# Superjie13/StereoTracking

Measured on AMD Instinct MI355X. Metric: stereo frame-pairs/sec @1280x720 D=192, higher is better.
Workload: dtype f32; 1 GPU; configs[1]: batch=8 synthetic 1280x720 stereo pairs per GPU, D=192, full YOLOX-s two-branch backbone+PAFPN+head, cost volume at 1/4 res (48 levels) + 2 3x3 aggregation convs + soft-argmin, decode+NMS, per-box depth; global_batch=8, inflight_contexts=4, distinct_input_batches=4, gpu_max_hw_queues=4, hip_force_dev_kernarg=1, parallelism=single process, no process group (no collective in the step), collectives_issued=0, tuning_plan=configs/tuning/mi355x.json, max_det=1000, detections_overflow=False

## Files before the change

include/stereotrack.h:

```cpp
#ifndef STEREOTRACK_H_
#define STEREOTRACK_H_

#include <stddef.h>
#include <stdint.h>

#ifdef __cplusplus
extern "C" {
#endif

#define ST_VERSION 430

enum {
  ST_OK = 0,
  ST_ERR_INVALID = -1,
  ST_ERR_HIP = -2,
  ST_ERR_STATE = -3,
  ST_ERR_WORKSPACE = -4,
  ST_ERR_NOTFOUND = -5
};

typedef void* st_stream_t;

int st_version(void);
const char* st_last_error(void);

typedef struct StConvDesc {
  const float* in_dev;
  int N, Hi, Wi, Cin, in_ld, in_off;
  const float* wgt_dev;
  const float* bias_dev;
  int Cout, KH, KW, stride, pad;
  float* out1_dev;
  int out1_ld, out1_off, split;
  float* out2_dev;
  int out2_ld, out2_off;
  float* up_dev;
  int up_ld, up_off;
  const float* res_dev;
  int res_ld, res_off;
  float post_scale;
  int act;
  const float* wgt_wino_dev;
} StConvDesc;

int st_conv2d_nhwc(const StConvDesc* d, st_stream_t stream);
int st_conv2d_nhwc_variant(const StConvDesc* d, st_stream_t stream, int variant);
size_t st_wino_packed_floats(int Cout, int Cin);
int st_wino_pack_weights(const float* packed_wgt_host, int Cout, int Cin, float* out_host);
int st_conv3x3_wino_group(const StConvDesc* descs, int n, st_stream_t stream);

int st_conv1x1_chain(const StConvDesc* a, const StConvDesc* b, st_stream_t stream);
size_t st_front_frag_floats(int Cout, int Cin);
int st_front_pack_frags(const float* packed_wgt_host, int Cout, int Cin, float* out_host);
int st_conv3x3s2_csp_front(const StConvDesc* a, const StConvDesc* ms, const StConvDesc* c1, const float* frag_ms_dev,
                           const float* frag_c1_dev, st_stream_t stream);
size_t st_csp_tail_frag_floats(void);
int st_csp_tail_pack_frags(const float* packed_wgt_host, float* out_host);
int st_conv3x3_csp_tail(const StConvDesc* conv2, const StConvDesc* fin, const float* frag_fin_dev, st_stream_t stream);
size_t st_conv_packed_floats(int Cout, int Cin, int KH, int KW);
int st_conv_pack_weights(const float* w, const float* conv_bias,
                         const float* bn_gamma, const float* bn_beta,
                         const float* bn_mean, const float* bn_var,
                         double bn_eps, int Cout, int Cin, int KH, int KW,
                         float* wgt_out, float* bias_out);

int st_focus_pack(const float* img_nchw_dev, int N, int C, int H, int W,
                  float* out_nhwc_dev, st_stream_t stream);

size_t st_stem_packed_floats(int Cout);
int st_stem_pack_weights(const float* w, const float* conv_bias,
                         const float* bn_gamma, const float* bn_beta,
                         const float* bn_mean, const float* bn_var,
                         double bn_eps, int Cout, int used_planes, float* wgt_out, float* bias_out);
int st_stem_focus_conv(const float* img_nchw_dev, int N, int H, int W, int used_planes, const float* wgt_dev,
                       const float* bias_dev, int Cout, float* out_nhwc_dev, int out_ld, int out_off,
                       int act , st_stream_t stream);
int st_stem_focus_conv_u8(const unsigned char* const* frames_u8_dev_ptrs_host, int N, int h, int w, int H, int W,
                          float pad_value, const float* wgt_dev, const float* bias_dev, int Cout, float* out_dev,
                          int out_ld, int out_off, int act, st_stream_t stream);

int st_pack_raw_inputs(const unsigned char* img_u8_dev, const unsigned short* disp_u16_dev, int N, int h, int w,
                       int H, int W, float img_pad, float* img_out_dev, float* disp_postp_out_dev,
// ... 415 lines not shown
```

stereotracking_amd/_lib.py:

```python
import ctypes as C
import os

import torch

_HERE = os.path.dirname(os.path.abspath(__file__))
LIB_PATH = os.path.join(_HERE, 'lib', 'libstereotrack_hip.so')

ST_OK = 0
_ERR_NAMES = {-1: 'ST_ERR_INVALID', -2: 'ST_ERR_HIP', -3: 'ST_ERR_STATE', -4: 'ST_ERR_WORKSPACE',
              -5: 'ST_ERR_NOTFOUND'}


class StError(RuntimeError):
    """A libstereotrack_hip call returned a non-zero status."""


class StConvDesc(C.Structure):
    _fields_ = [
        ('in_dev', C.c_void_p),
        ('N', C.c_int), ('Hi', C.c_int), ('Wi', C.c_int), ('Cin', C.c_int), ('in_ld', C.c_int), ('in_off', C.c_int),
        ('wgt_dev', C.c_void_p), ('bias_dev', C.c_void_p),
        ('Cout', C.c_int), ('KH', C.c_int), ('KW', C.c_int), ('stride', C.c_int), ('pad', C.c_int),
        ('out1_dev', C.c_void_p), ('out1_ld', C.c_int), ('out1_off', C.c_int), ('split', C.c_int),
        ('out2_dev', C.c_void_p), ('out2_ld', C.c_int), ('out2_off', C.c_int),
# ... 91 lines not shown
                ('wgt_reg_dev', C.c_void_p), ('bias_reg_dev', C.c_void_p),
                ('out_dev', C.c_void_p), ('M', C.c_int)]


class StDecodeDesc(C.Structure):
    _fields_ = [
        ('struct_size', C.c_int), ('batch', C.c_int), ('num_levels', C.c_int),
        ('level_h', C.c_int * 4), ('level_w', C.c_int * 4), ('level_stride', C.c_int * 4),
        ('level_offset', C.c_size_t * 4),
        ('score_thr', C.c_float), ('iou_thr', C.c_float), ('max_det', C.c_int),
        ('scale_x', C.c_float), ('scale_y', C.c_float), ('pad_left', C.c_float), ('pad_top', C.c_float),
        ('ori_w', C.c_float), ('ori_h', C.c_float), ('nms_mask_rows', C.c_int), ('num_classes', C.c_int),
        ('single_label', C.c_int),
    ]


_vp, _i, _f, _sz = C.c_void_p, C.c_int, C.c_float, C.c_size_t
_PROTOS = {
    'st_version': (C.c_int, []),
    'st_head_row_floats': (_i, [_i]),
    'st_png_unfilter': (_i, [_vp, _i, _i, _i, _vp]),
    'st_stem_focus_conv_u8': (_i, [_vp, _i, _i, _i, _i, _i, _f, _vp, _vp, _i, _vp, _i, _i, _i, _vp]),
    'st_detector_forward_raw': (_i, [_vp, _vp, _i, _i, _f, _vp, _vp, _sz, _vp, _vp]),
    'st_detector_forward_phase0_raw': (_i, [_vp, _vp, _vp, _i, _i, _f, _vp, _sz, _vp]),
    'st_pack_raw_frames': (_i, [_vp, _i, _i, _i, _i, _i, _f, _vp, _vp]),
    'st_resize_planes': (_i, [_vp, _i, _i, _i, _i, _vp, _i, _i, _i, _i, _vp]),
    'st_detector_set_split': (_i, [_vp, _i]),
    'st_split_instances_available': (_i, []),
    'st_volume_agg3d': (_i, [_vp, _vp, _i, _i, _i, _i, _vp, _f, _i, _vp]),
    'st_last_error': (C.c_char_p, []),
    'st_conv2d_nhwc': (_i, [C.POINTER(StConvDesc), _vp]),
    'st_conv2d_nhwc_variant': (_i, [C.POINTER(StConvDesc), _vp, _i]),
    'st_conv3x3_wino_group': (_i, [C.POINTER(StConvDesc), _i, _vp]),
    'st_head_pred': (_i, [C.POINTER(StHeadPredLevel), _i, _i, _vp]),
    'st_detector_op_owner': (_i, [_vp, _i, _vp, _vp]),
    'st_conv1x1_chain': (_i, [C.POINTER(StConvDesc), C.POINTER(StConvDesc), _vp]),
    'st_front_frag_floats': (_sz, [_i, _i]),
    'st_front_pack_frags': (_i, [_vp, _i, _i, _vp]),
    'st_conv3x3s2_csp_front': (_i, [C.POINTER(StConvDesc), C.POINTER(StConvDesc), C.POINTER(StConvDesc), _vp, _vp, _vp]),
    'st_csp_tail_frag_floats': (_sz, []),
    'st_csp_tail_pack_frags': (_i, [_vp, _vp]),
    'st_conv3x3_csp_tail': (_i, [C.POINTER(StConvDesc), C.POINTER(StConvDesc), _vp, _vp]),
    'st_conv_packed_floats': (_sz, [_i, _i, _i, _i]),
    'st_wino_packed_floats': (_sz, [_i, _i]),
    'st_wino_pack_weights': (_i, [_vp, _i, _i, _vp]),
    'st_conv_pack_weights': (_i, [_vp, _vp, _vp, _vp, _vp, _vp, C.c_double, _i, _i, _i, _i, _vp, _vp]),
    'st_focus_pack': (_i, [_vp, _i, _i, _i, _i, _vp, _vp]),
    'st_stem_packed_floats': (_sz, [_i]),
    'st_stem_pack_weights': (_i, [_vp, _vp, _vp, _vp, _vp, _vp, C.c_double, _i, _i, _vp, _vp]),
    'st_stem_focus_conv': (_i, [_vp, _i, _i, _i, _i, _vp, _vp, _i, _vp, _i, _i, _i, _vp]),
    'st_pack_raw_inputs': (_i, [_vp, _vp, _i, _i, _i, _i, _i, _f, _vp, _vp, _vp, _vp]),
    'st_spp_pool': (_i, [_vp, _i, _i, _i, _i, _i, _i, _vp, _i, _i, _vp]),
    'st_detector_create': (_i, [C.POINTER(StDetectorConfig), C.POINTER(_vp)]),
    'st_detector_destroy': (_i, [_vp]),
    'st_detector_num_params': (_i, [_vp]),
    'st_detector_param_info': (_i, [_vp, _i, C.c_char_p, _i, C.POINTER(C.c_int64), C.POINTER(_i)]),
    'st_detector_set_param': (_i, [_vp, C.c_char_p, _vp, C.c_int64]),
    'st_detector_finalize': (_i, [_vp]),
    'st_detector_workspace_bytes': (_sz, [_vp]),
    'st_detector_head_floats': (_sz, [_vp]),
    'st_detector_num_levels': (_i, [_vp]),
    'st_detector_level_info': (_i, [_vp, _i, C.POINTER(_i), C.POINTER(_i), C.POINTER(_i), C.POINTER(_sz)]),
    'st_detector_forward': (_i, [_vp, _vp, _vp, _vp, _sz, _vp, _vp]),
    'st_detector_forward_phase': (_i, [_vp, _i, _vp, _vp, _vp, _vp, _sz, _vp, _vp]),
    'st_detector_macs': (C.c_double, [_vp]),
    'st_detector_set_timing': (_i, [_vp, _i]),
# ... 121 lines not shown
```

stereotracking_amd/csrc/conv_igemm.hip:

```cpp
#include <algorithm>

#include <type_traits>

#include "st_common.h"

namespace st {

typedef float f32x16 __attribute__((ext_vector_type(16)));
typedef float f32x4 __attribute__((ext_vector_type(4)));
typedef unsigned int u32x4 __attribute__((ext_vector_type(4)));

struct ConvKArgs {
  const float* in;
  const float* wgt;
  const float* bias;
  float* out1;
  float* out2;
  float* up;
  const float* res;
  int Hi, Wi, Cin, in_ld, in_off;
  int Ho, Wo, HoWo, Cout;
  int KH, KW, stride, pad;
  int K, Kpad, M;
  unsigned in_bytes, wgt_bytes;
// ... 656 lines not shown
  return id >= 0 && id < kNumVariants && round_up(cout, 32) % kVariants[id].bn == 0;
}
const char* conv_variant_name(int id) {
  static const char* names[] = {"128x128", "128x64w2", "128x32w2", "64x64", "64x32w2",
                                "128x64", "128x32", "64x128", "256x64", "64x64w1", "64x32w1", "32x64w1",
                                "128x128dma", "64x64dma", "64x128dma", "128x32dma", "128x64dma",
                                "128x128dmab", "64x64dmab", "256x128dma", "256x128dmab", "256x128",
                                "128x128ws", "64x64ws", "64x128ws", "128x32ws", "128x64ws", "128x128ws2",
                                "64x128ws2", "128x128ws4"};
  return id >= 0 && id < kNumVariants ? names[id] : "-";
}

const char* conv_variant_signature(int id) {
  static const char* sigs[] = {"2, 2, 2, 2, 2, 1, 0", "2, 2, 2, 1, 2, 1, 0", "2, 1, 2, 1, 2, 1, 0",
                               "1, 1, 2, 2, 2, 1, 0", "1, 1, 2, 1, 2, 1, 0", "1, 2, 4, 1, 2, 1, 0",
                               "1, 1, 4, 1, 2, 1, 0", "1, 2, 2, 2, 2, 1, 0", "2, 2, 4, 1, 2, 1, 0",
                               "2, 2, 1, 1, 1, 1, 0", "2, 1, 1, 1, 1, 1, 0", "1, 2, 1, 1, 1, 1, 0",
                               "2, 2, 2, 2, 2, 1, 1", "1, 1, 2, 2, 2, 1, 1", "1, 2, 2, 2, 2, 1, 1",
                               "1, 1, 4, 1, 2, 1, 1", "1, 2, 4, 1, 2, 1, 1", "2, 2, 2, 2, 2, 0, 1",
                               "1, 1, 2, 2, 2, 0, 1", "2, 2, 4, 2, 2, 1, 1", "2, 2, 4, 2, 2, 0, 1",
                               "2, 2, 4, 2, 2, 1, 0", "ws 2, 2, 2, 2", "ws 1, 1, 2, 2", "ws 1, 2, 2, 2",
                               "ws 1, 1, 4, 1", "ws 1, 2, 4, 1", "ws 2, 2, 2, 2, 2", "ws 1, 2, 2, 2, 2",
                               "ws 2, 2, 2, 2, 4"};
  return id >= 0 && id < kNumVariants ? sigs[id] : "";
}

bool pw_conv_applicable(const StConvDesc& d);
int pw_conv_launch(const StConvDesc& d, hipStream_t stream, const StConvDesc* chain);
int pwr_conv_launch(const StConvDesc& d, hipStream_t stream, const StConvDesc* chain);
bool pwr_chain_applicable(const StConvDesc& d, const StConvDesc& c);
bool dc_conv_applicable(const StConvDesc& d);
int dc_conv_launch(const StConvDesc& d, hipStream_t stream);
bool wino_conv_applicable(const StConvDesc& d);
int wino_conv_launch(const StConvDesc& d, hipStream_t stream, bool narrow);
int wino_persist_launch(const StConvDesc& d, hipStream_t stream);

int conv2d_launch(const StConvDesc& d, hipStream_t stream, int force_variant, int* picked_variant) {
  ST_REQUIRE(d.in_dev && d.wgt_dev && d.bias_dev && d.out1_dev, "conv: null pointer");
  if (force_variant == 41) {
    if (picked_variant) *picked_variant = 41;
    return pw_conv_launch(d, stream, nullptr);
  }
  if (force_variant == 46) {
    if (picked_variant) *picked_variant = 46;
    return pwr_conv_launch(d, stream, nullptr);
  }
  if (force_variant == 42) {
    if (picked_variant) *picked_variant = 42;
    return dc_conv_launch(d, stream);
  }
  if (force_variant == 43 || force_variant == 44) {
    if (picked_variant) *picked_variant = force_variant;
    return wino_conv_launch(d, stream, force_variant == 44);
  }
#ifdef ST_ABLATION
  if (force_variant == 57) {
    if (picked_variant) *picked_variant = 57;
    return wino_persist_launch(d, stream);
  }
#endif
  ST_REQUIRE(d.Cin % 4 == 0 && d.in_ld % 4 == 0 && d.in_off % 4 == 0,
             "conv: Cin/in_ld/in_off must be multiples of 4 (got %d/%d/%d)", d.Cin, d.in_ld,
             d.in_off);
  ST_REQUIRE(d.N > 0 && d.Hi > 0 && d.Wi > 0 && d.Cout > 0 && d.KH > 0 && d.KW > 0 &&
                 d.stride > 0 && d.pad >= 0,
             "conv: bad geometry");
  ST_REQUIRE(d.in_off + d.Cin <= d.in_ld, "conv: input channel slice exceeds in_ld");
  const int Ho = (d.Hi + 2 * d.pad - d.KH) / d.stride + 1;
  const int Wo = (d.Wi + 2 * d.pad - d.KW) / d.stride + 1;
  ST_REQUIRE(Ho > 0 && Wo > 0, "conv: empty output");
  const int split = (d.out2_dev ? d.split : d.Cout);
  ST_REQUIRE(split >= 0 && split <= d.Cout, "conv: bad split");
  ST_REQUIRE(d.out1_off + split <= d.out1_ld, "conv: out1 slice exceeds out1_ld");
  if (d.out2_dev)
    ST_REQUIRE(d.out2_off + (d.Cout - split) <= d.out2_ld, "conv: out2 slice exceeds out2_ld");
  if (d.up_dev) ST_REQUIRE(d.up_off + d.Cout <= d.up_ld, "conv: up slice exceeds up_ld");
  if (d.res_dev) ST_REQUIRE(d.res_off + d.Cout <= d.res_ld, "conv: res slice exceeds res_ld");
  const long long M_ll = (long long)d.N * Ho * Wo;
  ST_REQUIRE(M_ll * (long long)std::max(std::max(d.out1_ld, d.out2_ld), d.res_dev ? d.res_ld : 1) < (1ll << 31) &&
                 (long long)d.N * d.Hi * d.Wi * d.in_ld < (1ll << 29) &&
                 d.KH * d.KW <= 32 &&
                 (!d.up_dev || 4 * M_ll * d.up_ld < (1ll << 31)),
             "conv: tensor exceeds 2^31 elements");
  ST_REQUIRE((long long)d.N * d.Hi * d.Wi < (1ll << 31) && M_ll < (1ll << 31),
             "conv: pixel count exceeds int32");

// ... 116 lines not shown
```

stereotracking_amd/csrc/wino_conv.hip:

```cpp
#include <algorithm>
#include <cmath>
#include <cstdint>
#include <cstdlib>
#include <cstring>
#include <vector>

#include "st_common.h"
#include "wino_pk.h"

namespace st {
namespace {

constexpr int WN_TX = 8, WN_TY = 4;
constexpr int WN_WW = 2 * WN_TX + 2, WN_WH = 2 * WN_TY + 2;
constexpr int WN_PIX = WN_WW * WN_WH;
constexpr int WN_PIECES = (WN_PIX + 7) / 8;
constexpr int WN_WIN_FLOATS = WN_PIECES * 8 * 32;
constexpr int wn_lds_floats(int cbn) {
  return 4 * 2 * 32 * 32 * cbn > 2 * WN_WIN_FLOATS ? 4 * 2 * 32 * 32 * cbn : 2 * WN_WIN_FLOATS;
}

struct WinoArgs {
  const float* in;
  const float* wino;
  const float* bias;
  float* out;
  const float* res;
  int N, H, W, Cin, in_ld, in_off, Cout;
  int out_ld, out_off, res_ld, res_off;
  float post_scale;
  int act;
  int tbx, tby, ncb, nkc;
  int g_last;
  unsigned nblocks, per_xcd, order, grid;
  unsigned in_bytes, out_bytes, res_bytes, wino_bytes;
};

template <int CBN, int LCBN, bool RES, bool KTAIL>
__device__ __forceinline__ void wino_conv3x3_body(const WinoArgs& p, int b_) {
  constexpr int WN_CB = 32 * CBN;
  constexpr int WN_FRAG_FLOATS = LCBN * 64 * 4;
  extern __shared__ float4 wn_smem4[];
  float* smem = reinterpret_cast<float*>(wn_smem4);
  const int tid = threadIdx.x, lane = tid & 63, a = tid >> 6;
  const int i = lane & 31, h = lane >> 5;
  const int tyi = i >> 3, txi = i & 7;
  const int cb = b_ % p.ncb; b_ /= p.ncb;
  const int bx = b_ % p.tbx; b_ /= p.tbx;
  const int by = b_ % p.tby;
  const int n = b_ / p.tby;
  const int wy0 = by * (2 * WN_TY) - 1, wx0 = bx * (2 * WN_TX) - 1;

#if defined(__HIP_DEVICE_COMPILE__)
  const __amdgpu_buffer_rsrc_t irsrc =
      __builtin_amdgcn_make_buffer_rsrc(const_cast<float*>(p.in), 0, (int)p.in_bytes, 0x00020000);
  const __amdgpu_buffer_rsrc_t wrsrc =
      __builtin_amdgcn_make_buffer_rsrc(const_cast<float*>(p.wino), 0, (int)p.wino_bytes, 0x00020000);
  const __amdgpu_buffer_rsrc_t orsrc = __builtin_amdgcn_make_buffer_rsrc(p.out, 0, (int)p.out_bytes, 0x00020000);
  const __amdgpu_buffer_rsrc_t rrsrc = __builtin_amdgcn_make_buffer_rsrc(
      const_cast<float*>(RES ? p.res : p.in), 0, (int)(RES ? p.res_bytes : 0u), 0x00020000);

  constexpr int NPW = (WN_PIECES + 3) / 4;
  unsigned poff[NPW];
  unsigned tail_ok = 0;
#pragma unroll
  for (int k = 0; k < NPW; ++k) {
    const int j = a + 4 * k;
    const int q = 8 * j + (lane >> 3), sl = lane & 7;
    const int wr = q / WN_WW, wc = q - wr * WN_WW;
    const int y = wy0 + wr, x = wx0 + wc;
    const bool ok = j < WN_PIECES && q < WN_PIX && y >= 0 && y < p.H && x >= 0 && x < p.W;
    const int quad = sl ^ ((q >> 1) & 7);
    poff[k] = ok ? (unsigned)((((n * p.H + y) * p.W + x) * p.in_ld + p.in_off + 4 * quad) * 4) : 0x80000000u;
    if ((p.nkc - 1) * 32 + 4 * quad < p.Cin) tail_ok |= 1u << k;
  }
  auto dma_window = [&](int kc, int buf) {
    const bool last = kc == p.nkc - 1;
#pragma unroll
    for (int k = 0; k < NPW; ++k) {
      const int j = a + 4 * k;
      const unsigned off = (last && !((tail_ok >> k) & 1u)) ? 0x80000000u : poff[k];
      if (j < WN_PIECES)
        __builtin_amdgcn_raw_ptr_buffer_load_lds(
            irsrc, (__attribute__((address_space(3))) void*)(smem + buf * WN_WIN_FLOATS + j * 256), 16, off,
            kc * 128, 0, 0);
    }
  };

  const int r0 = a == 0 ? 0 : (a == 2 ? 2 : 1);
  const int r1 = a == 0 ? 2 : (a == 1 ? 2 : (a == 2 ? 1 : 3));
  const f32x2 sgn = a == 1 ? f32x2{1.0f, 1.0f} : f32x2{-1.0f, -1.0f};
  int qoff[8], qsw[8];
#pragma unroll
  for (int k = 0; k < 8; ++k) {
    const int r = k < 4 ? r0 : r1, c = k & 3;
    const int q = (2 * tyi + r) * WN_WW + 2 * txi + c;
    qoff[k] = q * 32;
    qsw[k] = (q >> 1) & 7;
  }

  constexpr int SPLIT = LCBN / CBN;
  const unsigned wbase = (unsigned)(((((cb / SPLIT) * 4 + a) * p.nkc) * 16) * WN_FRAG_FLOATS + (cb % SPLIT) * CBN * 256 +
                                    lane * 4) * 4u;
  const int last_step = p.nkc * 16 - 1;
  auto load_frag = [&](int step, f32x4 (&f)[CBN]) {
    const int soff = (step < last_step ? step : last_step) * (WN_FRAG_FLOATS * 4);
#pragma unroll
    for (int nb = 0; nb < CBN; ++nb)
      f[nb] = __builtin_bit_cast(f32x4, __builtin_amdgcn_raw_buffer_load_b128(wrsrc, wbase, soff + 1024 * nb, 0));
  };

  f32x16 acc[4][CBN];
#pragma unroll
  for (int b = 0; b < 4; ++b)
#pragma unroll
    for (int nb = 0; nb < CBN; ++nb)
#pragma unroll
      for (int r = 0; r < 16; ++r) acc[b][nb][r] = 0.f;

  dma_window(0, 0);
  f32x4 fe[CBN], fo[CBN];
  load_frag(0, fe);
  asm volatile("s_waitcnt vmcnt(0)" ::: "memory");
  __syncthreads();

  for (int kc = 0; kc < p.nkc; ++kc) {
    const int buf = kc & 1;
    if (kc + 1 < p.nkc) dma_window(kc + 1, buf ^ 1);
    const float* win = smem + buf * WN_WIN_FLOATS;
    const int gn = (KTAIL && kc == p.nkc - 1) ? p.g_last : 4;
#pragma unroll
    for (int g = 0; g < 4; ++g) {
      if (KTAIL && g >= gn) continue;
      f32x4 d[8];
#pragma unroll
      for (int k = 0; k < 8; ++k)
        d[k] = *reinterpret_cast<const f32x4*>(win + qoff[k] + (((2 * g + h) ^ qsw[k]) << 2));
      f32x4 P[4], V[4];
#pragma unroll
      for (int c = 0; c < 4; ++c) P[c] = wn_addsgn(d[c], sgn, d[4 + c]);
      V[0] = wn_sub_mfma(P[0], P[2]);
      V[1] = wn_add_mfma(P[1], P[2]);
      V[2] = wn_sub_mfma(P[2], P[1]);
      V[3] = wn_sub_mfma(P[1], P[3]);
#pragma unroll
      for (int b = 0; b < 4; ++b) {
        const int step = (kc * 4 + g) * 4 + b;
        if (b & 1) load_frag(step + 1, fe); else load_frag(step + 1, fo);
#pragma unroll
        for (int s = 0; s < 4; ++s)
#pragma unroll
          for (int nb = 0; nb < CBN; ++nb)
            acc[b][nb] = __builtin_amdgcn_mfma_f32_32x32x2f32(V[b][s], (b & 1) ? fo[nb][s] : fe[nb][s], acc[b][nb],
                                                              0, 0, 0);
      }
    }
    asm volatile("s_waitcnt vmcnt(0)" ::: "memory");
    __syncthreads();
  }

  float* Rb = smem;
  __builtin_amdgcn_sched_barrier(0);
  asm volatile("s_nop 15\n\ts_nop 3" ::: "memory");
  __builtin_amdgcn_sched_barrier(0);
#pragma unroll
  for (int nb = 0; nb < CBN; ++nb)
#pragma unroll
    for (int r = 0; r < 16; ++r) {
      const int m = (r & 3) + 8 * (r >> 2) + 4 * h;
      if (r & 1) continue;
      const f32x2 a0{acc[0][nb][r], acc[0][nb][r + 1]}, a1{acc[1][nb][r], acc[1][nb][r + 1]};
      const f32x2 a2{acc[2][nb][r], acc[2][nb][r + 1]}, a3{acc[3][nb][r], acc[3][nb][r + 1]};
      const f32x2 R0 = wn_pk_add(wn_pk_add(a0, a1), a2);
      const f32x2 R1 = wn_pk_sub(wn_pk_sub(a1, a2), a3);
#pragma unroll
      for (int e = 0; e < 2; ++e) {
        Rb[((a * 2 + 0) * 32 + m + e) * WN_CB + nb * 32 + i] = R0[e];
        Rb[((a * 2 + 1) * 32 + m + e) * WN_CB + nb * 32 + i] = R1[e];
      }
    }
  __syncthreads();
  constexpr int LPT = WN_CB / 4;
  constexpr int TPI = 64 / LPT;
  const int c4 = (lane % LPT) * 4, tsel = lane / LPT;
  const int co = cb * WN_CB + c4;
  const f32x4 bias4 = *reinterpret_cast<const f32x4*>(p.bias + co);
  typedef unsigned u32x4 __attribute__((ext_vector_type(4)));
#pragma unroll
  for (int t8 = 0; t8 < 8; t8 += TPI) {
    const int txo = t8 + tsel;
    const int t = a * 8 + txo;
    const int oy0 = by * (2 * WN_TY) + 2 * a, ox0 = bx * (2 * WN_TX) + 2 * txo;
#pragma unroll
    for (int j = 0; j < 2; ++j) {
      const f32x4 q0 = *reinterpret_cast<const f32x4*>(Rb + ((0 * 2 + j) * 32 + t) * WN_CB + c4);
      const f32x4 q1 = *reinterpret_cast<const f32x4*>(Rb + ((1 * 2 + j) * 32 + t) * WN_CB + c4);
      const f32x4 q2 = *reinterpret_cast<const f32x4*>(Rb + ((2 * 2 + j) * 32 + t) * WN_CB + c4);
      const f32x4 q3 = *reinterpret_cast<const f32x4*>(Rb + ((3 * 2 + j) * 32 + t) * WN_CB + c4);
      const f32x4 y[2] = {wn_add(wn_add(q0, q1), q2), wn_sub(wn_sub(q1, q2), q3)};
#pragma unroll
      for (int ii = 0; ii < 2; ++ii) {
        const int oy = oy0 + ii, ox = ox0 + j;
        const bool ok = oy < p.H && ox < p.W && co < p.Cout;
        const int m = (n * p.H + oy) * p.W + ox;
        f32x4 v = wn_add(y[ii], bias4);
        if (p.act) {
#pragma unroll
          for (int e = 0; e < 4; ++e) v[e] = wn_silu(v[e]);
        }
        if (RES) {
          const unsigned roff = ok ? (unsigned)((m * p.res_ld + p.res_off + co) * 4) : 0x80000000u;
          const f32x4 rv = __builtin_bit_cast(f32x4, __builtin_amdgcn_raw_buffer_load_b128(rrsrc, roff, 0, 0));
#pragma unroll
          for (int e = 0; e < 4; ++e) v[e] = (v[e] + rv[e]) * p.post_scale;
        }
        const unsigned off = ok ? (unsigned)((m * p.out_ld + p.out_off + co) * 4) : 0x80000000u;
        __builtin_amdgcn_raw_buffer_store_b128(__builtin_bit_cast(u32x4, v), orsrc, off, 0, 0);
      }
    }
  }
#else
  (void)smem; (void)i; (void)h; (void)tyi; (void)txi; (void)cb; (void)n; (void)wy0; (void)wx0;
#endif
}

__device__ __forceinline__ bool wn_block_of(unsigned bid, unsigned order, unsigned per_xcd, unsigned ncb, unsigned nblocks,
                                            unsigned& b) {
  if (order == 2) {
    const unsigned slot = bid >> 3;
    b = ((slot / ncb) * 8u + (bid & 7u)) * ncb + slot % ncb;
  } else if (order == 1) {
    b = (bid & 7u) * per_xcd + (bid >> 3);
  } else {
    b = bid;
  }
  return b < nblocks;
}
static unsigned wn_order() {
#ifdef ST_ABLATION
  if (const char* e = getenv("ST_WINO_ORDER")) return (unsigned)atoi(e);
#endif
  return 0u;
}
static unsigned wn_grid(long long blocks, unsigned ncb, unsigned order, unsigned* per_xcd) {
  *per_xcd = (unsigned)((blocks + 7) / 8);
  if (order == 1) return 8u * *per_xcd;
  if (order == 2) return (unsigned)((blocks / ncb + 7) / 8 * 8 * ncb);
  return (unsigned)blocks;
}

template <int CBN, int LCBN, bool RES, bool KTAIL>
__global__ __launch_bounds__(256, 2) void wino_conv3x3_kernel(const WinoArgs p) {
  unsigned b;
  if (!wn_block_of(blockIdx.x, p.order, p.per_xcd, (unsigned)p.ncb, p.nblocks, b)) return;
  wino_conv3x3_body<CBN, LCBN, RES, KTAIL>(p, (int)b);
}

constexpr int WN_GROUP_MAX = 6;
struct WinoGroupArgs {
  WinoArgs p[WN_GROUP_MAX];
  unsigned first[WN_GROUP_MAX + 1];
  int n;
};

template <int CBN, int LCBN>
__global__ __launch_bounds__(256, 2) void wino_conv3x3_group_kernel(const WinoGroupArgs g) {
  const unsigned bid = blockIdx.x;
  int k = 0;
#pragma unroll
  for (int q = 1; q < WN_GROUP_MAX; ++q) k += (q < g.n && bid >= g.first[q]) ? 1 : 0;
  unsigned b;
  if (!wn_block_of(bid - g.first[k], g.p[k].order, g.p[k].per_xcd, (unsigned)g.p[k].ncb, g.p[k].nblocks, b)) return;
  wino_conv3x3_body<CBN, LCBN, false, false>(g.p[k], (int)b);
}


#ifdef ST_ABLATION
constexpr int wnp_lds_floats() { return 2 * WN_WIN_FLOATS + 4 * 2 * 32 * 32; }

template <int CBN, int LCBN, bool RES, bool KTAIL>
__global__ __launch_bounds__(256, 2) void wino_conv3x3_persist_kernel(const WinoArgs p) {
#if defined(__HIP_DEVICE_COMPILE__)
  constexpr int WN_FRAG_FLOATS = LCBN * 64 * 4;
  constexpr int SPLIT = LCBN / CBN;
  extern __shared__ float4 wn_smem4[];
  float* smem = reinterpret_cast<float*>(wn_smem4);
  float* Rb = smem + 2 * WN_WIN_FLOATS;
  const int tid = threadIdx.x, lane = tid & 63, a = tid >> 6;
  const int i = lane & 31, h = lane >> 5;
  const int tyi = i >> 3, txi = i & 7;
  const __amdgpu_buffer_rsrc_t irsrc =
      __builtin_amdgcn_make_buffer_rsrc(const_cast<float*>(p.in), 0, (int)p.in_bytes, 0x00020000);
  const __amdgpu_buffer_rsrc_t wrsrc =
      __builtin_amdgcn_make_buffer_rsrc(const_cast<float*>(p.wino), 0, (int)p.wino_bytes, 0x00020000);
  const __amdgpu_buffer_rsrc_t orsrc = __builtin_amdgcn_make_buffer_rsrc(p.out, 0, (int)p.out_bytes, 0x00020000);
  const __amdgpu_buffer_rsrc_t rrsrc = __builtin_amdgcn_make_buffer_rsrc(
      const_cast<float*>(RES ? p.res : p.in), 0, (int)(RES ? p.res_bytes : 0u), 0x00020000);
  constexpr int NPW = (WN_PIECES + 3) / 4;

  auto block_of = [&](unsigned b, int& cb, int& bx, int& by, int& n) {
    cb = (int)(b % (unsigned)p.ncb); b /= (unsigned)p.ncb;
    bx = (int)(b % (unsigned)p.tbx); b /= (unsigned)p.tbx;
    by = (int)(b % (unsigned)p.tby);
    n = (int)(b / (unsigned)p.tby);
  };
  unsigned tail_ok = 0;
// ... 215 lines not shown
    for (int a = 0; a < 4; ++a)
      for (int kc = 0; kc < nkc; ++kc)
        for (int g = 0; g < 4; ++g)
          for (int b = 0; b < 4; ++b)
            for (int nb = 0; nb < cbn; ++nb)
              for (int l = 0; l < 64; ++l)
                for (int e = 0; e < 4; ++e) {
                  const int j = l & 31, h = l >> 5;
                  const int co = cb * CB + nb * 32 + j, ci = kc * 32 + 8 * g + 4 * h + e;
                  double u = 0.0;
                  if (co < Cout && ci < Cin)
                    for (int kh = 0; kh < 3; ++kh)
                      for (int kw = 0; kw < 3; ++kw)
                        u += G[a][kh] * (double)packed[(size_t)co * Kpad + (kh * 3 + kw) * Cin + ci] * G[b][kw];
                  out[(((((((size_t)cb * 4 + a) * nkc + kc) * 4 + g) * 4 + b) * cbn + nb) * 64 + l) * 4 + e] = (float)u;
                }
  return ST_OK;
}

bool wino_conv_applicable(const StConvDesc& d) {
  if (!d.wgt_wino_dev) return false;
  if (d.KH != 3 || d.KW != 3 || d.stride != 1 || d.pad != 1 || d.up_dev || d.out2_dev) return false;
  if (!wino_shape_ok(d.Cin, d.Cout)) return false;
  if ((d.in_ld | d.in_off | d.out1_ld | d.out1_off) & 3) return false;
  if ((reinterpret_cast<uintptr_t>(d.in_dev) | reinterpret_cast<uintptr_t>(d.out1_dev)) & 15) return false;
  if (d.res_dev && (((d.res_ld | d.res_off) & 3) || (reinterpret_cast<uintptr_t>(d.res_dev) & 15))) return false;
  if (d.Cout % 4) return false;
  const long long M = (long long)d.N * d.Hi * d.Wi, lim = 1ll << 31;
  if (M * d.in_ld * 4 >= lim || M * d.out1_ld * 4 >= lim) return false;
  if (d.res_dev && M * d.res_ld * 4 >= lim) return false;
  return true;
}

template <int CBN, int LCBN, bool RES, bool KTAIL = false>
static int wino_launch_instance(const WinoArgs& a, unsigned blocks, hipStream_t stream) {
  constexpr int lds = wn_lds_floats(CBN) * (int)sizeof(float);
  static int lds_set = 0;
  auto kern = wino_conv3x3_kernel<CBN, LCBN, RES, KTAIL>;
  ST_ENSURE_DYNAMIC_LDS(kern, lds, lds_set);
  hipLaunchKernelGGL(kern, dim3(a.grid), dim3(256), lds, stream, a);
  return ST_OK;
}

static int wino_fill_args(const StConvDesc& d, bool narrow, WinoArgs& a, long long* blocks_out) {
  ST_REQUIRE(wino_conv_applicable(d), "winograd conv: shape not supported (3x3 s1 p1, Cin % 4 == 0, Cout a multiple of 32 "
                                      "or <= 64, transformed weights required)");
  ST_REQUIRE(d.in_dev && d.bias_dev && d.out1_dev, "winograd conv: null pointer");
  ST_REQUIRE(d.in_off + d.Cin <= d.in_ld && d.out1_off + d.Cout <= d.out1_ld, "winograd conv: channel slice exceeds ld");
  if (d.res_dev) ST_REQUIRE(d.res_off + d.Cout <= d.res_ld, "winograd conv: res slice exceeds res_ld");
  const long long M = (long long)d.N * d.Hi * d.Wi;
  const int lcbn = wino_cbn(d.Cout);
  ST_REQUIRE(!narrow || (lcbn == 2 && d.Cout % 64 == 0), "winograd conv: the narrow instance needs Cout %% 64 == 0");
  const int cbn = narrow ? 1 : lcbn, CB = 32 * cbn;
  a.in = d.in_dev; a.wino = d.wgt_wino_dev; a.bias = d.bias_dev; a.out = d.out1_dev; a.res = d.res_dev;
  a.N = d.N; a.H = d.Hi; a.W = d.Wi; a.Cin = d.Cin; a.in_ld = d.in_ld; a.in_off = d.in_off; a.Cout = d.Cout;
  a.out_ld = d.out1_ld; a.out_off = d.out1_off; a.res_ld = d.res_ld; a.res_off = d.res_off;
  a.post_scale = d.res_dev ? d.post_scale : 1.0f;
  a.act = d.act;
  a.tbx = ceil_div(d.Wi, 2 * WN_TX); a.tby = ceil_div(d.Hi, 2 * WN_TY);
  a.ncb = round_up(d.Cout, CB) / CB; a.nkc = round_up(d.Cin, 32) / 32;
  a.in_bytes = (unsigned)(M * d.in_ld * 4);
  a.out_bytes = (unsigned)(M * d.out1_ld * 4);
  a.res_bytes = d.res_dev ? (unsigned)(M * d.res_ld * 4) : 0u;
  a.wino_bytes = (unsigned)(wino_packed_floats(d.Cout, d.Cin) * 4);
  a.g_last = 4 - (a.nkc * 32 - d.Cin) / 8;
  const long long blocks = (long long)d.N * a.tbx * a.tby * a.ncb;
  ST_REQUIRE(blocks + 8 < (1ll << 31), "winograd conv: grid too large");
  a.nblocks = (unsigned)blocks;
  a.order = wn_order();
  a.grid = wn_grid(blocks, (unsigned)a.ncb, a.order, &a.per_xcd);
  *blocks_out = blocks;
  return ST_OK;
}

int wino_conv_launch(const StConvDesc& d, hipStream_t stream, bool narrow) {
  WinoArgs a;
  long long blocks = 0;
  ST_CHECK(wino_fill_args(d, narrow, a, &blocks));
  const int lcbn = wino_cbn(d.Cout);
  const int cbn = narrow ? 1 : lcbn;
  const bool ktail = a.g_last < 4;
  int rc;
  if (ktail && cbn == 2 && !d.res_dev) rc = wino_launch_instance<2, 2, false, true>(a, (unsigned)blocks, stream);
  else if (ktail && cbn == 1 && lcbn == 1 && !d.res_dev) rc = wino_launch_instance<1, 1, false, true>(a, (unsigned)blocks, stream);
  else if (cbn == 2) rc = d.res_dev ? wino_launch_instance<2, 2, true>(a, (unsigned)blocks, stream)
                               : wino_launch_instance<2, 2, false>(a, (unsigned)blocks, stream);
  else if (lcbn == 2) rc = d.res_dev ? wino_launch_instance<1, 2, true>(a, (unsigned)blocks, stream)
                                     : wino_launch_instance<1, 2, false>(a, (unsigned)blocks, stream);
  else rc = d.res_dev ? wino_launch_instance<1, 1, true>(a, (unsigned)blocks, stream)
                      : wino_launch_instance<1, 1, false>(a, (unsigned)blocks, stream);
  ST_CHECK(rc);
  ST_CHECK_HIP(hipGetLastError());
  return ST_OK;
}


#ifdef ST_ABLATION
bool wino_persist_applicable(const StConvDesc& d) { return wino_conv_applicable(d) && wino_cbn(d.Cout) == 2; }

template <int CBN, int LCBN, bool RES, bool KTAIL>
static int wino_persist_instance(const WinoArgs& a, unsigned grid, hipStream_t stream) {
  constexpr int lds = wnp_lds_floats() * (int)sizeof(float);
  static int lds_set = 0;
  auto kern = wino_conv3x3_persist_kernel<CBN, LCBN, RES, KTAIL>;
  ST_ENSURE_DYNAMIC_LDS(kern, lds, lds_set);
  hipLaunchKernelGGL(kern, dim3(grid), dim3(256), lds, stream, a);
  return ST_OK;
}

int wino_persist_launch(const StConvDesc& d, hipStream_t stream) {
  ST_REQUIRE(wino_persist_applicable(d), "winograd conv (persistent): needs a Winograd layer with the 64-cout layout");
  WinoArgs a;
  long long blocks = 0;
  ST_CHECK(wino_fill_args(d, false, a, &blocks));
  static int cus = 0;
  if (cus == 0) {
    int dev = 0, n = 0;
    ST_CHECK_HIP(hipGetDevice(&dev));
    ST_CHECK_HIP(hipDeviceGetAttribute(&n, hipDeviceAttributeMultiprocessorCount, dev));
    cus = std::max(1, n);
  }
  const unsigned grid = (unsigned)std::min<long long>(blocks, 2ll * cus);
  const bool ktail = a.g_last < 4;
  int rc;
  if (ktail) rc = d.res_dev ? wino_persist_instance<2, 2, true, true>(a, grid, stream)
                            : wino_persist_instance<2, 2, false, true>(a, grid, stream);
  else rc = d.res_dev ? wino_persist_instance<2, 2, true, false>(a, grid, stream)
                      : wino_persist_instance<2, 2, false, false>(a, grid, stream);
  ST_CHECK(rc);
  ST_CHECK_HIP(hipGetLastError());
  return ST_OK;
}

#endif

bool wino_group_applicable(const StConvDesc* d, int n) {
  if (n < 2 || n > WN_GROUP_MAX) return false;
  for (int k = 0; k < n; ++k)
    if (!wino_conv_applicable(d[k]) || d[k].res_dev || d[k].Cout % 64 != 0 || d[k].Cin % 32 != 0) return false;
  return true;
}

int wino_group_launch(const StConvDesc* d, int n, hipStream_t stream) {
  ST_REQUIRE(wino_group_applicable(d, n), "winograd group: layers do not qualify (3x3 s1 p1, Cout %% 64 == 0, Cin %% 32 "
                                          "== 0, no residual, 2..%d layers)", WN_GROUP_MAX);
  WinoGroupArgs g;
  std::memset(&g, 0, sizeof(g));
  g.n = n;
  long long total = 0;
  for (int k = 0; k < n; ++k) {
    long long blocks = 0;
    ST_CHECK(wino_fill_args(d[k], false, g.p[k], &blocks));
    g.first[k] = (unsigned)total;
    total += (g.p[k].grid + 7u) / 8u * 8u;
    ST_REQUIRE(total + 8 < (1ll << 31), "winograd group: grid too large");
  }
  for (int k = n; k <= WN_GROUP_MAX; ++k) g.first[k] = (unsigned)total;
  constexpr int lds = wn_lds_floats(2) * (int)sizeof(float);
  static int lds_set = 0;
  auto kern = wino_conv3x3_group_kernel<2, 2>;
  ST_ENSURE_DYNAMIC_LDS(kern, lds, lds_set);
  hipLaunchKernelGGL(kern, dim3((unsigned)total), dim3(256), lds, stream, g);
  ST_CHECK_HIP(hipGetLastError());
  return ST_OK;
}

}

extern "C" int st_conv3x3_wino_group(const StConvDesc* descs, int n, st_stream_t stream) {
  if (!descs) return st::set_error(ST_ERR_INVALID, "st_conv3x3_wino_group: null descriptors");
  return st::wino_group_launch(descs, n, static_cast<hipStream_t>(stream));
}

extern "C" size_t st_wino_packed_floats(int Cout, int Cin) { return st::wino_packed_floats(Cout, Cin); }

extern "C" int st_wino_pack_weights(const float* packed_wgt_host, int Cout, int Cin, float* out_host) {
  return st::wino_pack_weights(packed_wgt_host, Cout, Cin, out_host);
}
```

Measured before the change: 1787 stereo frame-pairs/s.

## Add shape-adaptive Winograd tile blockings that pack multiple sub-tiles per block

Generalizes the Winograd 3x3 conv kernel so each 32-tile block can cover G smaller sub-regions (e.g. 2x 8x4 tiles) instead of one fixed 8x4 region, chosen per layer by minimizing padded tile slots for the map size. This targets wasted work from edge tiles on small or oddly shaped feature maps, especially in grouped launches. It adds per-thread selection arithmetic for the sub-block origin and more template instances, and a larger halo overhead per useful pixel when G > 1.

```diff
diff --git a/include/stereotrack.h b/include/stereotrack.h
--- a/include/stereotrack.h
+++ b/include/stereotrack.h
@@ -48,6 +48,9 @@
 size_t st_wino_packed_floats(int Cout, int Cin);
 int st_wino_pack_weights(const float* packed_wgt_host, int Cout, int Cin, float* out_host);
 int st_conv3x3_wino_group(const StConvDesc* descs, int n, st_stream_t stream);
+int st_conv3x3_wino_blocked(const StConvDesc* d, st_stream_t stream, int narrow, int blocking);
+int st_wino_pick_blocking(int H, int W, int* tile_slots);
+int st_wino_blocking_slots(int H, int W, int blocking);
 
 int st_conv1x1_chain(const StConvDesc* a, const StConvDesc* b, st_stream_t stream);
 size_t st_front_frag_floats(int Cout, int Cin);
diff --git a/stereotracking_amd/_lib.py b/stereotracking_amd/_lib.py
--- a/stereotracking_amd/_lib.py
+++ b/stereotracking_amd/_lib.py
@@ -147,6 +147,9 @@
     'st_conv2d_nhwc': (_i, [C.POINTER(StConvDesc), _vp]),
     'st_conv2d_nhwc_variant': (_i, [C.POINTER(StConvDesc), _vp, _i]),
     'st_conv3x3_wino_group': (_i, [C.POINTER(StConvDesc), _i, _vp]),
+    'st_conv3x3_wino_blocked': (_i, [C.POINTER(StConvDesc), _vp, _i, _i]),
+    'st_wino_pick_blocking': (_i, [_i, _i, C.POINTER(_i)]),
+    'st_wino_blocking_slots': (_i, [_i, _i, _i]),
     'st_head_pred': (_i, [C.POINTER(StHeadPredLevel), _i, _i, _vp]),
     'st_detector_op_owner': (_i, [_vp, _i, _vp, _vp]),
     'st_conv1x1_chain': (_i, [C.POINTER(StConvDesc), C.POINTER(StConvDesc), _vp]),
diff --git a/stereotracking_amd/csrc/conv_igemm.hip b/stereotracking_amd/csrc/conv_igemm.hip
--- a/stereotracking_amd/csrc/conv_igemm.hip
+++ b/stereotracking_amd/csrc/conv_igemm.hip
@@ -712,7 +712,7 @@
 bool dc_conv_applicable(const StConvDesc& d);
 int dc_conv_launch(const StConvDesc& d, hipStream_t stream);
 bool wino_conv_applicable(const StConvDesc& d);
-int wino_conv_launch(const StConvDesc& d, hipStream_t stream, bool narrow);
+int wino_conv_launch(const StConvDesc& d, hipStream_t stream, bool narrow, int blocking);
 int wino_persist_launch(const StConvDesc& d, hipStream_t stream);
 
 int conv2d_launch(const StConvDesc& d, hipStream_t stream, int force_variant, int* picked_variant) {
@@ -731,7 +731,7 @@
   }
   if (force_variant == 43 || force_variant == 44) {
     if (picked_variant) *picked_variant = force_variant;
-    return wino_conv_launch(d, stream, force_variant == 44);
+    return wino_conv_launch(d, stream, force_variant == 44, -1);
   }
 #ifdef ST_ABLATION
   if (force_variant == 57) {
diff --git a/stereotracking_amd/csrc/wino_conv.hip b/stereotracking_amd/csrc/wino_conv.hip
--- a/stereotracking_amd/csrc/wino_conv.hip
+++ b/stereotracking_amd/csrc/wino_conv.hip
@@ -15,10 +15,14 @@
 constexpr int WN_WW = 2 * WN_TX + 2, WN_WH = 2 * WN_TY + 2;
 constexpr int WN_PIX = WN_WW * WN_WH;
 constexpr int WN_PIECES = (WN_PIX + 7) / 8;
-constexpr int WN_WIN_FLOATS = WN_PIECES * 8 * 32;
-constexpr int wn_lds_floats(int cbn) {
-  return 4 * 2 * 32 * 32 * cbn > 2 * WN_WIN_FLOATS ? 4 * 2 * 32 * 32 * cbn : 2 * WN_WIN_FLOATS;
-}
+[[maybe_unused]] constexpr int WN_WIN_FLOATS = WN_PIECES * 8 * 32;
+
+struct WnBlocking { int G, lsy, lsx; };
+constexpr int WN_NBLK = 4;
+constexpr WnBlocking WN_BLK[WN_NBLK] = {{1, 2, 3}, {2, 1, 3}, {4, 0, 3}, {2, 2, 2}};
+constexpr int wn_blk_wpix(int k) { return (2 * (1 << WN_BLK[k].lsy) + 2) * (2 * (1 << WN_BLK[k].lsx) + 2); }
+constexpr int wn_blk_pieces(int k) { return (WN_BLK[k].G * wn_blk_wpix(k) + 7) / 8; }
+static_assert(wn_blk_pieces(0) == WN_PIECES && wn_blk_wpix(0) == WN_PIX, "blocking A is the 18 x 10 window");
 
 struct WinoArgs {
   const float* in;
@@ -31,25 +35,50 @@
   float post_scale;
   int act;
   int tbx, tby, ncb, nkc;
+  int blk, sbx, sby;
   int g_last;
   unsigned nblocks, per_xcd, order, grid;
   unsigned in_bytes, out_bytes, res_bytes, wino_bytes;
 };
 
-template <int CBN, int LCBN, bool RES, bool KTAIL>
+template <int CBN, int LCBN, bool RES, bool KTAIL, int BLK>
 __device__ __forceinline__ void wino_conv3x3_body(const WinoArgs& p, int b_) {
+  constexpr int G = WN_BLK[BLK].G, LSY = WN_BLK[BLK].lsy, LSX = WN_BLK[BLK].lsx;
+  constexpr int WW = (2 << LSX) + 2, WPIX = wn_blk_wpix(BLK);
+  constexpr int PIECES = wn_blk_pieces(BLK), WIN_FLOATS = PIECES * 8 * 32;
   constexpr int WN_CB = 32 * CBN;
   constexpr int WN_FRAG_FLOATS = LCBN * 64 * 4;
   extern __shared__ float4 wn_smem4[];
   float* smem = reinterpret_cast<float*>(wn_smem4);
   const int tid = threadIdx.x, lane = tid & 63, a = tid >> 6;
   const int i = lane & 31, h = lane >> 5;
-  const int tyi = i >> 3, txi = i & 7;
   const int cb = b_ % p.ncb; b_ /= p.ncb;
-  const int bx = b_ % p.tbx; b_ /= p.tbx;
-  const int by = b_ % p.tby;
-  const int n = b_ / p.tby;
-  const int wy0 = by * (2 * WN_TY) - 1, wx0 = bx * (2 * WN_TX) - 1;
+  int sbyx[G], sbpix[G];
+  {
+    const int s = b_ * G;
+    int sc = s % p.sbx, sr = s / p.sbx;
+    int sn = sr / p.sby;
+    sr -= sn * p.sby;
+#pragma unroll
+    for (int gi = 0; gi < G; ++gi) {
+      const bool present = sn < p.N;
+      const int y0 = present ? sr << (LSY + 1) : p.H + 1, x0 = sc << (LSX + 1);
+      sbyx[gi] = (y0 << 16) | x0;
+      sbpix[gi] = present ? ((sn * p.H + y0) * p.W + x0) : 0;
+      if (++sc == p.sbx) {
+        sc = 0;
+        if (++sr == p.sby) { sr = 0; ++sn; }
+      }
+    }
+  }
+  auto sb_sel = [](const int (&v)[G], int gi) {
+    int r = v[0];
+#pragma unroll
+    for (int k = 1; k < G; ++k) r += (v[k] - v[k - 1]) & -(int)(gi >= k);
+    return r;
+  };
+  constexpr int LSYX = LSY + LSX, TYMASK = (1 << LSY) - 1, TXMASK = (1 << LSX) - 1;
+  const int tgi = i >> LSYX, tyi = (i >> LSX) & TYMASK, txi = i & TXMASK;
 
 #if defined(__HIP_DEVICE_COMPILE__)
   const __amdgpu_buffer_rsrc_t irsrc =
@@ -60,18 +89,21 @@
   const __amdgpu_buffer_rsrc_t rrsrc = __builtin_amdgcn_make_buffer_rsrc(
       const_cast<float*>(RES ? p.res : p.in), 0, (int)(RES ? p.res_bytes : 0u), 0x00020000);
 
-  constexpr int NPW = (WN_PIECES + 3) / 4;
+  constexpr int NPW = (PIECES + 3) / 4;
   unsigned poff[NPW];
   unsigned tail_ok = 0;
 #pragma unroll
   for (int k = 0; k < NPW; ++k) {
     const int j = a + 4 * k;
     const int q = 8 * j + (lane >> 3), sl = lane & 7;
-    const int wr = q / WN_WW, wc = q - wr * WN_WW;
-    const int y = wy0 + wr, x = wx0 + wc;
-    const bool ok = j < WN_PIECES && q < WN_PIX && y >= 0 && y < p.H && x >= 0 && x < p.W;
+    const int gi = q / WPIX, qs = q - gi * WPIX;
+    const int wr = qs / WW, wc = qs - wr * WW;
+    const int yx = sb_sel(sbyx, gi);
+    const int y = (yx >> 16) - 1 + wr, x = (yx & 0xffff) - 1 + wc;
+    const bool ok = (j < PIECES) & (q < G * WPIX) & (y >= 0) & (y < p.H) & (x >= 0) & (x < p.W);
     const int quad = sl ^ ((q >> 1) & 7);
-    poff[k] = ok ? (unsigned)((((n * p.H + y) * p.W + x) * p.in_ld + p.in_off + 4 * quad) * 4) : 0x80000000u;
+    poff[k] = ok ? (unsigned)(((sb_sel(sbpix, gi) + (wr - 1) * p.W + wc - 1) * p.in_ld + p.in_off + 4 * quad) * 4)
+                 : 0x80000000u;
     if ((p.nkc - 1) * 32 + 4 * quad < p.Cin) tail_ok |= 1u << k;
   }
   auto dma_window = [&](int kc, int buf) {
@@ -80,9 +112,9 @@
     for (int k = 0; k < NPW; ++k) {
       const int j = a + 4 * k;
       const unsigned off = (last && !((tail_ok >> k) & 1u)) ? 0x80000000u : poff[k];
-      if (j < WN_PIECES)
+      if (j < PIECES)
         __builtin_amdgcn_raw_ptr_buffer_load_lds(
-            irsrc, (__attribute__((address_space(3))) void*)(smem + buf * WN_WIN_FLOATS + j * 256), 16, off,
+            irsrc, (__attribute__((address_space(3))) void*)(smem + buf * WIN_FLOATS + j * 256), 16, off,
             kc * 128, 0, 0);
     }
   };
@@ -94,7 +126,7 @@
 #pragma unroll
   for (int k = 0; k < 8; ++k) {
     const int r = k < 4 ? r0 : r1, c = k & 3;
-    const int q = (2 * tyi + r) * WN_WW + 2 * txi + c;
+    const int q = tgi * WPIX + (2 * tyi + r) * WW + 2 * txi + c;
     qoff[k] = q * 32;
     qsw[k] = (q >> 1) & 7;
   }
@@ -127,7 +159,7 @@
   for (int kc = 0; kc < p.nkc; ++kc) {
     const int buf = kc & 1;
     if (kc + 1 < p.nkc) dma_window(kc + 1, buf ^ 1);
-    const float* win = smem + buf * WN_WIN_FLOATS;
+    const float* win = smem + buf * WIN_FLOATS;
     const int gn = (KTAIL && kc == p.nkc - 1) ? p.g_last : 4;
 #pragma unroll
     for (int g = 0; g < 4; ++g) {
@@ -190,7 +222,10 @@
   for (int t8 = 0; t8 < 8; t8 += TPI) {
     const int txo = t8 + tsel;
     const int t = a * 8 + txo;
-    const int oy0 = by * (2 * WN_TY) + 2 * a, ox0 = bx * (2 * WN_TX) + 2 * txo;
+    const int ogi = t >> LSYX;
+    const int oty = 2 * ((t >> LSX) & TYMASK), otx = 2 * (t & TXMASK), oyx = sb_sel(sbyx, ogi);
+    const int oy0 = (oyx >> 16) + oty, ox0 = (oyx & 0xffff) + otx;
+    const int m0 = sb_sel(sbpix, ogi) + oty * p.W + otx;
 #pragma unroll
     for (int j = 0; j < 2; ++j) {
       const f32x4 q0 = *reinterpret_cast<const f32x4*>(Rb + ((0 * 2 + j) * 32 + t) * WN_CB + c4);
@@ -202,7 +237,7 @@
       for (int ii = 0; ii < 2; ++ii) {
         const int oy = oy0 + ii, ox = ox0 + j;
         const bool ok = oy < p.H && ox < p.W && co < p.Cout;
-        const int m = (n * p.H + oy) * p.W + ox;
+        const int m = m0 + ii * p.W + j;
         f32x4 v = wn_add(y[ii], bias4);
         if (p.act) {
 #pragma unroll
@@ -220,7 +255,7 @@
     }
   }
 #else
-  (void)smem; (void)i; (void)h; (void)tyi; (void)txi; (void)cb; (void)n; (void)wy0; (void)wx0;
+  (void)smem; (void)h; (void)tgi; (void)tyi; (void)txi; (void)cb; (void)sb_sel; (void)sbyx; (void)sbpix; (void)WW; (void)WPIX; (void)WIN_FLOATS;
 #endif
 }
 
@@ -249,11 +284,11 @@
   return (unsigned)blocks;
 }
 
-template <int CBN, int LCBN, bool RES, bool KTAIL>
+template <int CBN, int LCBN, bool RES, bool KTAIL, int BLK>
 __global__ __launch_bounds__(256, 2) void wino_conv3x3_kernel(const WinoArgs p) {
   unsigned b;
   if (!wn_block_of(blockIdx.x, p.order, p.per_xcd, (unsigned)p.ncb, p.nblocks, b)) return;
-  wino_conv3x3_body<CBN, LCBN, RES, KTAIL>(p, (int)b);
+  wino_conv3x3_body<CBN, LCBN, RES, KTAIL, BLK>(p, (int)b);
 }
 
 constexpr int WN_GROUP_MAX = 6;
@@ -271,7 +306,14 @@
   for (int q = 1; q < WN_GROUP_MAX; ++q) k += (q < g.n && bid >= g.first[q]) ? 1 : 0;
   unsigned b;
   if (!wn_block_of(bid - g.first[k], g.p[k].order, g.p[k].per_xcd, (unsigned)g.p[k].ncb, g.p[k].nblocks, b)) return;
-  wino_conv3x3_body<CBN, LCBN, false, false>(g.p[k], (int)b);
+  switch (g.p[k].blk) {
+    case 1: wino_conv3x3_body<CBN, LCBN, false, false, 1>(g.p[k], (int)b); break;
+#ifdef ST_ABLATION
+    case 2: wino_conv3x3_body<CBN, LCBN, false, false, 2>(g.p[k], (int)b); break;
+    case 3: wino_conv3x3_body<CBN, LCBN, false, false, 3>(g.p[k], (int)b); break;
+#endif
+    default: wino_conv3x3_body<CBN, LCBN, false, false, 0>(g.p[k], (int)b); break;
+  }
 }
 
 
@@ -553,17 +595,57 @@
   return true;
 }
 
-template <int CBN, int LCBN, bool RES, bool KTAIL = false>
-static int wino_launch_instance(const WinoArgs& a, unsigned blocks, hipStream_t stream) {
-  constexpr int lds = wn_lds_floats(CBN) * (int)sizeof(float);
+int wino_blocking_slots(int H, int W, int blocking) {
+  const WnBlocking& b = WN_BLK[blocking];
+  return ceil_div(H, 2 << b.lsy) * ceil_div(W, 2 << b.lsx) * (32 / b.G);
+}
+constexpr unsigned WN_BLK_SHIPPED = 0x3u;
+int wino_pick_blocking(int H, int W, unsigned allowed) {
+  int best = 0;
+  for (int k = 1; k < WN_NBLK; ++k) {
+    if (!((allowed >> k) & 1u)) continue;
+    const int s = wino_blocking_slots(H, W, k), sb = wino_blocking_slots(H, W, best);
+    if (s < sb || (s == sb && WN_BLK[k].G * wn_blk_wpix(k) < WN_BLK[best].G * wn_blk_wpix(best))) best = k;
+  }
+  return best;
+}
+static int wn_resolve_blocking(int requested, int H, int W) {
+  if (requested >= 0) return requested;
+  unsigned allowed = WN_BLK_SHIPPED;
+#ifdef ST_ABLATION
+  if (const char* e = getenv("ST_WINO_BLOCKING")) {
+    const int v = atoi(e);
+    if (v >= 0 && v < WN_NBLK) return v;
+  }
+  if (const char* e = getenv("ST_WINO_BLOCKING_MASK")) allowed = (unsigned)atoi(e);
+#endif
+  return wino_pick_blocking(H, W, allowed);
+}
+static int wn_lds_bytes(int blk, int cbn) {
+  return std::max(4 * 2 * 32 * 32 * cbn, 2 * wn_blk_pieces(blk) * 8 * 32) * (int)sizeof(float);
+}
+
+template <int CBN, int LCBN, bool RES, bool KTAIL, int BLK>
+static int wino_launch_blocked(const WinoArgs& a, hipStream_t stream) {
+  const int lds = wn_lds_bytes(BLK, CBN);
   static int lds_set = 0;
-  auto kern = wino_conv3x3_kernel<CBN, LCBN, RES, KTAIL>;
+  auto kern = wino_conv3x3_kernel<CBN, LCBN, RES, KTAIL, BLK>;
   ST_ENSURE_DYNAMIC_LDS(kern, lds, lds_set);
   hipLaunchKernelGGL(kern, dim3(a.grid), dim3(256), lds, stream, a);
   return ST_OK;
 }
-
-static int wino_fill_args(const StConvDesc& d, bool narrow, WinoArgs& a, long long* blocks_out) {
+template <int CBN, int LCBN, bool RES, bool KTAIL = false>
+static int wino_launch_instance(const WinoArgs& a, unsigned blocks, hipStream_t stream) {
+  switch (a.blk) {
+    case 0: return wino_launch_blocked<CBN, LCBN, RES, KTAIL, 0>(a, stream);
+    case 1: return wino_launch_blocked<CBN, LCBN, RES, KTAIL, 1>(a, stream);
+    case 2: return wino_launch_blocked<CBN, LCBN, RES, KTAIL, 2>(a, stream);
+    case 3: return wino_launch_blocked<CBN, LCBN, RES, KTAIL, 3>(a, stream);
+  }
+  return set_error(ST_ERR_INVALID, "winograd conv: unknown blocking %d", a.blk);
+}
+
+static int wino_fill_args(const StConvDesc& d, bool narrow, int blocking, WinoArgs& a, long long* blocks_out) {
   ST_REQUIRE(wino_conv_applicable(d), "winograd conv: shape not supported (3x3 s1 p1, Cin % 4 == 0, Cout a multiple of 32 "
                                       "or <= 64, transformed weights required)");
   ST_REQUIRE(d.in_dev && d.bias_dev && d.out1_dev, "winograd conv: null pointer");
@@ -585,7 +667,12 @@
   a.res_bytes = d.res_dev ? (unsigned)(M * d.res_ld * 4) : 0u;
   a.wino_bytes = (unsigned)(wino_packed_floats(d.Cout, d.Cin) * 4);
   a.g_last = 4 - (a.nkc * 32 - d.Cin) / 8;
-  const long long blocks = (long long)d.N * a.tbx * a.tby * a.ncb;
+  ST_REQUIRE(blocking >= -1 && blocking < WN_NBLK, "winograd conv: unknown blocking %d (-1 = picked, 0..3 = A..D)", blocking);
+  const int bk = wn_resolve_blocking(blocking, d.Hi, d.Wi);
+  const WnBlocking& B = WN_BLK[bk];
+  a.blk = bk;
+  a.sbx = ceil_div(d.Wi, 2 << B.lsx); a.sby = ceil_div(d.Hi, 2 << B.lsy);
+  const long long blocks = ((long long)d.N * a.sbx * a.sby + B.G - 1) / B.G * a.ncb;
   ST_REQUIRE(blocks + 8 < (1ll << 31), "winograd conv: grid too large");
   a.nblocks = (unsigned)blocks;
   a.order = wn_order();
@@ -594,10 +681,10 @@
   return ST_OK;
 }
 
-int wino_conv_launch(const StConvDesc& d, hipStream_t stream, bool narrow) {
+int wino_conv_launch(const StConvDesc& d, hipStream_t stream, bool narrow, int blocking) {
   WinoArgs a;
   long long blocks = 0;
-  ST_CHECK(wino_fill_args(d, narrow, a, &blocks));
+  ST_CHECK(wino_fill_args(d, narrow, blocking, a, &blocks));
   const int lcbn = wino_cbn(d.Cout);
   const int cbn = narrow ? 1 : lcbn;
   const bool ktail = a.g_last < 4;
@@ -633,7 +720,7 @@
   ST_REQUIRE(wino_persist_applicable(d), "winograd conv (persistent): needs a Winograd layer with the 64-cout layout");
   WinoArgs a;
   long long blocks = 0;
-  ST_CHECK(wino_fill_args(d, false, a, &blocks));
+  ST_CHECK(wino_fill_args(d, false, 0, a, &blocks));
   static int cus = 0;
   if (cus == 0) {
     int dev = 0, n = 0;
@@ -669,15 +756,19 @@
   std::memset(&g, 0, sizeof(g));
   g.n = n;
   long long total = 0;
+  int lds = 0;
   for (int k = 0; k < n; ++k) {
     long long blocks = 0;
-    ST_CHECK(wino_fill_args(d[k], false, g.p[k], &blocks));
+    ST_CHECK(wino_fill_args(d[k], false, -1, g.p[k], &blocks));
+#ifndef ST_ABLATION
+    ST_REQUIRE((WN_BLK_SHIPPED >> g.p[k].blk) & 1u, "winograd group: blocking %d is not a shipped one", g.p[k].blk);
+#endif
+    lds = std::max(lds, wn_lds_bytes(g.p[k].blk, 2));
     g.first[k] = (unsigned)total;
     total += (g.p[k].grid + 7u) / 8u * 8u;
     ST_REQUIRE(total + 8 < (1ll << 31), "winograd group: grid too large");
   }
   for (int k = n; k <= WN_GROUP_MAX; ++k) g.first[k] = (unsigned)total;
-  constexpr int lds = wn_lds_floats(2) * (int)sizeof(float);
   static int lds_set = 0;
   auto kern = wino_conv3x3_group_kernel<2, 2>;
   ST_ENSURE_DYNAMIC_LDS(kern, lds, lds_set);
@@ -693,6 +784,24 @@
   return st::wino_group_launch(descs, n, static_cast<hipStream_t>(stream));
 }
 
+extern "C" int st_conv3x3_wino_blocked(const StConvDesc* d, st_stream_t stream, int narrow, int blocking) {
+  if (!d) return st::set_error(ST_ERR_INVALID, "st_conv3x3_wino_blocked: null descriptor");
+  return st::wino_conv_launch(*d, static_cast<hipStream_t>(stream), narrow != 0, blocking);
+}
+
+extern "C" int st_wino_pick_blocking(int H, int W, int* tile_slots) {
+  if (H <= 0 || W <= 0) return st::set_error(ST_ERR_INVALID, "st_wino_pick_blocking: empty map %d x %d", H, W);
+  const int k = st::wino_pick_blocking(H, W, st::WN_BLK_SHIPPED);
+  if (tile_slots) *tile_slots = st::wino_blocking_slots(H, W, k);
+  return k;
+}
+
+extern "C" int st_wino_blocking_slots(int H, int W, int blocking) {
+  if (H <= 0 || W <= 0 || blocking < 0 || blocking >= st::WN_NBLK)
+    return st::set_error(ST_ERR_INVALID, "st_wino_blocking_slots: bad map %d x %d or blocking %d", H, W, blocking);
+  return st::wino_blocking_slots(H, W, blocking);
+}
+
 extern "C" size_t st_wino_packed_floats(int Cout, int Cin) { return st::wino_packed_floats(Cout, Cin); }
 
 extern "C" int st_wino_pack_weights(const float* packed_wgt_host, int Cout, int Cin, float* out_host) {
```

Result: no change. 1793 stereo frame-pairs/s, median of 6 (+0.3%).
